# TRI-ML/sdflabel

Measured on AMD Instinct MI355X. Metric: rendered rays/sec (fwd+bwd), higher is better.
Workload: dtype f32; 1 GPU; BASELINE configs[1]: one 256x256 crop(s) per GPU, DeepSDF 8x512 on a 40^3 grid, fwd+bwd to yaw/trans/latent, decoder re-evaluated every step; crops_per_gpu=1, rays_per_crop=65536, grid_points=64000, surfels=2751, front_facing=763, parallelism=crop-parallel x1

## Files before the change

### include/sdfr.h

```cpp
#ifndef SDFR_H
#define SDFR_H

#include <stdint.h>

#ifdef __cplusplus
extern "C" {
#endif

#define SDFR_OK 0
#define SDFR_E_INVALID (-1)
#define SDFR_E_HIP (-2)
#define SDFR_E_UNSUPPORTED (-3)

#define SDFR_MAX_LAYERS 16
#define SDFR_TRACE_LEVELS 6
#define SDFR_TRACE_COUNTERS 32

#define SDFR_VERSION 415

int sdfr_version(void);
int sdfr_build_flags(void);
const char* sdfr_last_error(void);

typedef struct sdfr_decoder sdfr_decoder;

int sdfr_decoder_create(sdfr_decoder** out, int n_lin, const int* in_dim, const int* out_dim,
                        const int* inj_n, const int* inj_off, const float* const* h_W, const float* const* h_b,
                        const float* const* h_ln_w, const float* const* h_ln_b, int n_inputs, int use_tanh, int device);
int sdfr_decoder_destroy(sdfr_decoder* dec);
int64_t sdfr_decoder_macs(const sdfr_decoder* dec);

int sdfr_mlp_forward(const sdfr_decoder* dec, const float* inputs, int64_t n, float* sdf,
                     uint32_t* mask_ws ,
                     void* stream);
int sdfr_grid_tile_order(int D, int32_t* out);
int sdfr_mlp_forward_ordered(const sdfr_decoder* dec, const float* inputs, int64_t n, float* sdf, uint32_t* mask_ws, const int32_t* order,
                             int64_t order_rows, void* stream);
int sdfr_mlp_forward_f16(const sdfr_decoder* dec, const float* inputs, int64_t n, float* sdf, uint32_t* mask_ws, void* stream);

int sdfr_mlp_forward_f16_counted(const sdfr_decoder* dec, const float* inputs, int64_t n_max, const int32_t* n_dev, float* sdf, uint32_t* mask_ws,
                                 void* stream);

int sdfr_mlp_forward_split(const sdfr_decoder* dec, const float* inputs, int64_t n, float* sdf, uint32_t* mask_ws, void* stream);
int sdfr_mlp_forward_split_counted(const sdfr_decoder* dec, const float* inputs, int64_t n_max, const int32_t* n_dev, float* sdf, void* stream);
int64_t sdfr_decoder_mask_words(const sdfr_decoder* dec, int64_t n);

int sdfr_mlp_jacobian(const sdfr_decoder* dec, const float* inputs, int64_t rows_per_crop, int B,
                      const int32_t* idx, int cap, const int32_t* cnt, float* J, float* sdf_sel,
                      const float* sdf_full ,
                      const uint32_t* mask_ws ,
                      int mask_from_f16 ,
                      void* stream);
// ... 340 lines not shown
                     const int32_t* windows, const int64_t* poff, int64_t P, const int32_t* triangle, const int32_t* owner, const int32_t* scene,
                     const int32_t* boxes, const int64_t* qoff, int64_t Q, const double* paint, const double* light, int S, const int32_t* bg_index,
                     const uint8_t* bg, int NBG, const int32_t* ramp, int B, int W, int H, const double* K, float z_min, uint8_t* rgb, int32_t* flags,
                     void* stream);

int64_t sdfr_mesh_sdf_ws_bytes(int B, int64_t N, int64_t T);
int sdfr_mesh_sdf(const float* vertices, int64_t V, const int32_t* faces, int64_t T, const int64_t* voff, const int64_t* toff,
                  const float* points, int64_t N, const int64_t* qoff, int B, int want_sign, void* ws, int64_t ws_bytes, float* sdf, float* dist,
                  double* d2, int32_t* nearest, double* winding, int32_t* flags, void* stream);
int64_t sdfr_mesh_surface_ws_bytes(int B, int64_t T);
int sdfr_mesh_surface_points(const float* vertices, int64_t V, const int32_t* faces, int64_t T, const int64_t* voff, const int64_t* toff,
                             const float* uniforms, int64_t S, const int64_t* soff, int B, void* ws, int64_t ws_bytes, float* points,
                             int32_t* triangle, int32_t* flags, void* stream);

int sdfr_debug_set_trace(void* device_buffer);

#ifdef __cplusplus
}
#endif
#endif
```

### sdflabel_amd/_lib.py

```python
import ctypes
import os
from ctypes import POINTER, c_char_p, c_float, c_int, c_int32, c_int64, c_void_p

_HERE = os.path.dirname(os.path.abspath(__file__))
LIB_PATH = os.environ.get("SDFR_LIB") or os.path.join(_HERE, "lib", "libsdfr_hip.so")

ABI_VERSION = 415
_lib = None

_PROTOS = {
    "sdfr_version": (c_int, []),
    "sdfr_build_flags": (c_int, []),
    "sdfr_last_error": (c_char_p, []),
    "sdfr_debug_set_trace": (c_int, [c_void_p]),
    "sdfr_mlp_forward_counted": (c_int, [c_void_p, c_void_p, c_int64, c_void_p, c_void_p, c_int, c_void_p]),
    "sdfr_trace_setup": (c_int, [c_void_p, c_void_p, c_void_p, c_int, c_int, c_int, c_int, c_float, c_float, c_void_p, c_void_p, c_void_p,
                                 c_void_p, c_void_p, c_void_p, c_int, c_void_p]),
    "sdfr_trace_setup2": (c_int, [c_void_p, c_void_p, c_void_p, c_int, c_int, c_int, c_int, c_float, c_float, c_void_p, c_void_p, c_void_p,
                                  c_void_p, c_void_p, c_void_p, c_int, c_void_p, c_void_p, c_void_p]),
    "sdfr_trace_cone": (c_int, [c_void_p, c_void_p, c_void_p, c_void_p, c_int, c_int, c_int, c_int, c_float, c_float, c_float, c_int, c_int,
                                c_int, c_float, c_int, c_void_p, c_void_p, c_void_p, c_void_p, c_void_p, c_void_p, c_void_p, c_void_p, c_void_p,
                                c_void_p, c_void_p]),
    "sdfr_trace_step": (c_int, [c_void_p, c_void_p, c_void_p, c_int, c_int, c_int, c_float, c_void_p, c_void_p, c_int, c_int64, c_void_p,
                                c_void_p, c_void_p, c_void_p, c_void_p, c_void_p, c_void_p, c_void_p, c_void_p]),
    "sdfr_trace_march": (c_int, [c_void_p, c_void_p, c_void_p, c_void_p, c_int, c_int, c_int, c_int, c_float, c_int, c_int, c_int, c_void_p, c_int,
                                 c_float, c_float, c_int, c_void_p, c_void_p, c_void_p, c_void_p, c_void_p, c_void_p, c_void_p, c_void_p,
                                 c_void_p, c_void_p, c_void_p, c_void_p, c_void_p, c_void_p]),
    "sdfr_trace_pool": (c_int, []),
    "sdfr_trace_hits": (c_int, [c_void_p, c_void_p, c_void_p, c_int, c_int, c_int, c_int, c_void_p, c_void_p, c_void_p, c_void_p, c_void_p, c_void_p]),
# ... 29 lines not shown
                                      c_void_p, c_void_p, c_void_p, c_void_p, c_void_p, c_void_p, c_void_p, c_void_p, c_void_p, c_void_p, c_void_p,
                                      c_void_p, c_void_p]),
    "sdfr_loss_2d_r": (c_int, [c_void_p, c_void_p, c_int, c_void_p, c_int, c_int, c_float, c_float, c_float, c_void_p, c_void_p, c_void_p,
                               c_void_p, c_void_p]),
    "sdfr_prefilter_audit_select": (c_int, [c_void_p, c_void_p, c_int64, c_int, c_int, c_int, c_void_p, c_void_p, c_void_p, c_void_p, c_int, c_void_p]),
    "sdfr_prefilter_audit_check": (c_int, [c_void_p, c_void_p, c_void_p, c_void_p, c_int, c_int64, c_int, c_float, c_void_p, c_void_p, c_void_p,
                                           c_void_p, c_void_p]),
    "sdfr_scale_net": (c_int, [c_void_p, c_int, c_void_p, c_void_p, c_void_p, c_void_p, c_void_p, c_void_p, c_void_p, c_void_p]),
    "sdfr_decoder_create": (c_int, [POINTER(c_void_p), c_int, POINTER(c_int), POINTER(c_int), POINTER(c_int), POINTER(c_int),
                                    POINTER(c_void_p), POINTER(c_void_p), POINTER(c_void_p), POINTER(c_void_p), c_int, c_int, c_int]),
    "sdfr_decoder_destroy": (c_int, [c_void_p]),
    "sdfr_decoder_macs": (c_int64, [c_void_p]),
    "sdfr_mlp_forward": (c_int, [c_void_p, c_void_p, c_int64, c_void_p, c_void_p, c_void_p]),
    "sdfr_grid_tile_order": (c_int, [c_int, c_void_p]),
    "sdfr_mlp_forward_ordered": (c_int, [c_void_p, c_void_p, c_int64, c_void_p, c_void_p, c_void_p, c_int64, c_void_p]),
    "sdfr_mlp_forward_f16": (c_int, [c_void_p, c_void_p, c_int64, c_void_p, c_void_p, c_void_p]),
    "sdfr_mlp_forward_f16_counted": (c_int, [c_void_p, c_void_p, c_int64, c_void_p, c_void_p, c_void_p, c_void_p]),
    "sdfr_mlp_forward_split": (c_int, [c_void_p, c_void_p, c_int64, c_void_p, c_void_p, c_void_p]),
    "sdfr_mlp_forward_split_counted": (c_int, [c_void_p, c_void_p, c_int64, c_void_p, c_void_p, c_void_p]),
    "sdfr_decoder_mask_words": (c_int64, [c_void_p, c_int64]),
    "sdfr_mlp_jacobian": (c_int, [c_void_p, c_void_p, c_int64, c_int, c_void_p, c_int, c_void_p, c_void_p, c_void_p, c_void_p,
                                  c_void_p, c_int, c_void_p]),
    "sdfr_band_select": (c_int, [c_void_p, c_int64, c_int, c_float, c_void_p, c_int, c_void_p, c_void_p, c_void_p, c_void_p]),
    "sdfr_band_select_margin": (c_int, [c_void_p, c_int64, c_int, c_float, c_void_p, c_void_p, c_int, c_void_p, c_void_p, c_void_p, c_void_p]),
    "sdfr_prefilter_guard": (c_int, [c_void_p, c_void_p, c_void_p, c_int64, c_int, c_int, c_void_p, c_void_p, c_void_p, c_void_p, c_void_p]),
    "sdfr_prefilter_plan": (c_int, [c_void_p, c_int64, c_int, c_int, c_int, c_float, c_void_p, c_void_p, c_void_p, c_void_p, c_int, c_void_p, c_void_p,
                                    c_void_p]),
    "sdfr_mlp_forward_f16_skip": (c_int, [c_void_p, c_void_p, c_int64, c_void_p, c_void_p, c_int64, c_void_p]),
    "sdfr_band_select_skip": (c_int, [c_void_p, c_int64, c_int, c_float, c_void_p, c_void_p, c_void_p, c_int, c_void_p, c_void_p, c_void_p, c_void_p]),
    "sdfr_prefilter_guard2": (c_int, [c_void_p, c_void_p, c_void_p, c_int64, c_int, c_int, c_void_p, c_void_p, c_void_p, c_void_p, c_void_p, c_void_p]),
# ... 188 lines not shown
    return torch._C._cuda_getCurrentRawStream(torch._C._cuda_getDevice())


class _NoGuard:
    def __enter__(self):
        return None

    def __exit__(self, *exc):
        return False


_NO_GUARD = _NoGuard()


TRAFFIC_SOURCES = {
    "traffic_mlp_forward.json": ("mlp_kernel.h", "kc_slots.h", "mlp.hip", "mlp_fwd32.hip"),
    "traffic_splat.json": ("splat.hip", "splat_bbox.h"),
    "traffic_sphere_step.json": ("trace.hip",),
}


def source_sha16(names):
    import hashlib
    h = hashlib.sha256()
    for n in names:
        with open(os.path.join(os.path.dirname(os.path.abspath(__file__)), "csrc", n), "rb") as f:
            h.update(n.encode() + b"\0" + f.read())
    return h.hexdigest()[:16]


def stored_traffic(root, name):
# ... 49 lines not shown
```

### sdflabel_amd/batch.py

```python
import math
import os

import torch

from . import _lib
from .grid import Grid3D

_DIAM_DISC = 0.04
_DEPTH_CONSTANT = 150.0
P, ck = _lib.ptr, _lib.check


class BatchRenderer:
    def __init__(self, decoder, density, K, resolution_px, batch, cap=None, device="cuda", threshold=0.03, output_nocs=True,
                 max_pixels=None, max_side=None, candidate_reuse=None):
        dev = torch.device(device)
        if dev.type != "cuda":
            raise _lib.SdfrError("BatchRenderer runs on the GPU only")
        self.dev, self.B = dev, int(batch)
        self._f = lambda *shape: torch.zeros(shape, dtype=torch.float32, device=dev)
        self._i = lambda *shape: torch.zeros(shape, dtype=torch.int32, device=dev)
        self.W, self.H = int(resolution_px[0]), int(resolution_px[1])
        self.thr = float(threshold)
        self.nocs_mode = 1 if output_nocs else 0
# ... 1 lines not shown
            raise NotImplementedError("BatchRenderer composites NOCS colours (the optimizer's configuration)")
        self.decoder = decoder
        prec = getattr(decoder, "mlp_precision", torch.float32)
        self.f16, self.split, self.prefilter = prec == torch.float16, prec == "float32_split", prec == "float32_prefilter"
        self.margin = float(getattr(decoder, "prefilter_margin", 0.005))
        self.handle = decoder.handle(dev)
        self.fused = bool(getattr(decoder, "fused_launches", True))
        self.L, self.NI = decoder.latent_size, decoder.latent_size + 3
        self.grid = Grid3D(density, dev).points.detach().contiguous()
        self.G = self.grid.shape[0]
        self.fwd_order = None
        if prec == torch.float32 and self.handle.hp == 512 and not self.handle.has_ln and self.G == int(density) ** 3:
            order = torch.empty(self.G, dtype=torch.int32)
            ck(_lib.lib().sdfr_grid_tile_order(int(density), P(order)), "sdfr_grid_tile_order")
            self.fwd_order = order.to(dev)
        self.cap = int(cap) if cap is not None else max(256, self.G // 8)
        self._init_extents(K, max_pixels, max_side)
        self._alloc_common()
        want_reuse = bool(getattr(decoder, "candidate_reuse", False)) if candidate_reuse is None else bool(candidate_reuse)
        self.creuse = (self.f16 or prec == torch.float32) and want_reuse and self.handle.hp == 512 and not self.handle.has_ln
        self.reuse_off_reason = None
        if want_reuse and not self.creuse:
            self.reuse_off_reason = "candidate reuse needs a float16 / float32 decoder of padded width 512 without LayerNorm"
        if self.prefilter:
            self._setup_prefilter(decoder)
        elif self.creuse:
            self._setup_candidate_reuse(decoder)
        self.mode = "prefilter" if self.prefilter else ("creuse" if self.creuse else "plain")
        self.guarded = self.prefilter or self.creuse
        self.n_full = self._i(self.B) if self.guarded else None
# ... 236 lines not shown
        return {"color": self.color, "mask": self.mask, "depth": self.depth, "normals": self.nimg, "xyzf": self.xyzf, "nf": self.fcnt, "n": self.cnt}

    def _params_stage(self, L, st, frozen):
        B, G = self.B, self.G
        if self.creuse and self.fused and not frozen:
            ck(L.sdfr_params_plan(P(self.yaw), P(self.trans), P(self.latent), self.L, P(self.grid), G, B, P(self.inputs), P(self.pose), P(self.latnorm),
                                  self.lipschitz_plan, P(self.margin_dev), P(self.max_dev), P(self.lat_ref), P(self.age), self.max_reuse, P(self.reuse_flag),
                                  P(self.n_full), st), "sdfr_params_plan")
        else:
            ck(L.sdfr_params_forward(P(self.yaw), P(self.trans), P(self.latent), self.L, P(self.grid), G, B, None if frozen else P(self.inputs),
                                     P(self.pose), P(self.latnorm), st), "sdfr_params_forward")

    def _decoder_plain(self, L, st, mlp_events, events):
        B, G, cap = self.B, self.G, self.cap
        fwd = L.sdfr_mlp_forward_f16 if self.f16 else (L.sdfr_mlp_forward_split if self.split else L.sdfr_mlp_forward)
        if self.fwd_order is not None and os.environ.get("SDFR_FWD_ORDER", "1") != "0":
            ck(L.sdfr_mlp_forward_ordered(self.handle.h, P(self.inputs), B * G, P(self.sdf), P(self.mask_ws), P(self.fwd_order), G, st),
               "sdfr_mlp_forward_ordered")
        else:
            ck(fwd(self.handle.h, P(self.inputs), B * G, P(self.sdf), P(self.mask_ws), st), fwd.__name__)
        if mlp_events is not None:
            mlp_events[1].record()
        ck(L.sdfr_band_select_ex(P(self.sdf), G, B, self.thr, None, None, P(self.idx), cap, P(self.cnt), None, P(self.scratch), P(self.over), 1, st),
           "sdfr_band_select_ex")
        if "jacobian" in events:
            events["jacobian"][0].record()
        ck(L.sdfr_mlp_jacobian(self.handle.h, P(self.inputs), G, B, P(self.idx), cap, P(self.cnt), P(self.J), P(self.sdf_band), P(self.sdf),
                               P(self.mask_ws), 2 if self.f16 else 0, st), "sdfr_mlp_jacobian")
        if "jacobian" in events:
            events["jacobian"][1].record()

# ... 241 lines not shown
```

### sdflabel_amd/csrc/mlp.hip

```cpp
#include "mlp_kernel.h"
#include <algorithm>
#include <cmath>
#include <stdlib.h>
#include <string.h>
#include <vector>


#define SDFR_DEVICE_CHECK(d, what)                                                                                                          \
    do {                                                                                                                                    \
        int cur_ = -1;                                                                                                                      \
        SDFR_HIP_CHECK(hipGetDevice(&cur_));                                                                                                \
        SDFR_REQUIRE(cur_ == (d)->device, "%s: the decoder's weights live on device %d but the current device (the launch stream's) is %d: " \
                     "create one decoder handle per device", what, (d)->device, cur_);                                                      \
    } while (0)

extern "C" int sdfr_decoder_create(sdfr_decoder** out, int n_lin, const int* in_dim, const int* out_dim,
                                   const int* inj_n, const int* inj_off, const float* const* h_W,
                                   const float* const* h_b, const float* const* h_ln_w, const float* const* h_ln_b, int n_inputs,
                                   int use_tanh, int device) {
    SDFR_REQUIRE(out && in_dim && out_dim && inj_n && inj_off && h_W && h_b, "sdfr_decoder_create: NULL argument");
    SDFR_REQUIRE(n_lin >= 2 && n_lin <= SDFR_MAX_LAYERS, "sdfr_decoder_create: n_lin=%d outside [2,%d]", n_lin, SDFR_MAX_LAYERS);
    SDFR_REQUIRE(out_dim[n_lin - 1] == 1, "sdfr_decoder_create: last layer must have out_dim 1 (got %d)", out_dim[n_lin - 1]);
    SDFR_REQUIRE(in_dim[0] == n_inputs && inj_n[0] == 0, "sdfr_decoder_create: layer 0 must consume exactly the input row");
    int width = 0;
// ... 115 lines not shown
        P.kcompact = finite ? 1 : 0;
    }
    if (!Wkj.empty()) {
        SDFR_HIP_CHECK(hipMalloc(&d->d_Wkj, Wkj.size() * sizeof(float)));
        SDFR_HIP_CHECK(hipMemcpy(d->d_Wkj, Wkj.data(), Wkj.size() * sizeof(float), hipMemcpyHostToDevice));
        P.Wkj = d->d_Wkj;
        P.jcompact = finite ? 1 : 0;
    }
    P.Wf = d->d_Wf; P.Wb = d->d_Wb; P.Wh = d->d_Wh; P.Ws = d->d_Ws; P.Wbh = d->d_Wbh; P.bias = d->d_bias; P.w_last = d->d_wlast; P.fwd_np = 2;
    *out = d;
    return SDFR_OK;
}

static unsigned long long* g_trace = nullptr;
extern "C" int sdfr_debug_set_trace(void* device_buffer) { g_trace = (unsigned long long*)device_buffer; return SDFR_OK; }

extern "C" int sdfr_decoder_destroy(sdfr_decoder* d) {
    if (!d) return SDFR_OK;
    void* bufs[] = {d->d_Wf, d->d_Wb, d->d_Wk, d->d_Wkj, d->d_Wh, d->d_Ws, d->d_Wbh, d->d_bias, d->d_wlast, d->d_lng, d->d_lnb, d->ln_ws};
    for (void* b : bufs) (void)hipFree(b);
    delete d;
    return SDFR_OK;
}

extern "C" int64_t sdfr_decoder_macs(const sdfr_decoder* d) { return d ? d->macs : 0; }

static void mask_geometry(int HP, int* ft, int* nt) {
    if (HP == 128) { *ft = 1; *nt = 256; }
    else if (HP == 256) { *ft = 2; *nt = 256; }
    else { *ft = 2; *nt = 512; }
// ... 1 lines not shown

extern "C" int64_t sdfr_decoder_mask_words(const sdfr_decoder* d, int64_t n) {
    if (!d || n <= 0) return 0;
    int ft, nt;
    mask_geometry(d->HP, &ft, &nt);
    return ((n + 127) / 128) * 2 * (int64_t)(d->n_lin - 1) * ft * nt;
}

extern "C" int sdfr_mlp_forward(const sdfr_decoder* d, const float* inputs, int64_t n, float* sdf, uint32_t* mask_ws, void* stream) {
    SDFR_REQUIRE(d && inputs && sdf, "sdfr_mlp_forward: NULL argument");
    SDFR_DEVICE_CHECK(d, "sdfr_mlp_forward");
    SDFR_REQUIRE(n >= 0 && n < (int64_t)1 << 31, "sdfr_mlp_forward: n=%lld out of range", (long long)n);
    if (n == 0) return SDFR_OK;
    MlpParams P = d->proto;
    P.inputs = inputs; P.n = n; P.sdf = sdf; P.maskbuf = mask_ws; P.trace = g_trace;
    const int grid = sdfr_cdiv(n, 64);
    if (d->has_ln) sdfr_launch_ln(P, d->HP, false, grid, 1, (hipStream_t)stream);
    else if (d->HP == 512) sdfr_launch_fwd_f32_512(P, n, mask_ws != nullptr, (hipStream_t)stream);
    else sdfr_launch_small(P, d->HP, mask_ws ? 1 : 0, grid, 1, (hipStream_t)stream);
    SDFR_LAUNCH_CHECK();
    return SDFR_OK;
}

extern "C" int sdfr_grid_tile_order(int D, int32_t* out) {
    SDFR_REQUIRE(out, "sdfr_grid_tile_order: NULL argument");
    SDFR_REQUIRE(D >= 1 && D <= 1024, "sdfr_grid_tile_order: D=%d outside [1,1024]", D);
    int64_t j = 0;
    for (int bx = 0; bx < D; bx += 4)
        for (int by = 0; by < D; by += 4)
            for (int bz = 0; bz < D; bz += 4)
// ... 5 lines not shown

extern "C" int sdfr_mlp_forward_ordered(const sdfr_decoder* d, const float* inputs, int64_t n, float* sdf, uint32_t* mask_ws, const int32_t* order,
                                        int64_t order_rows, void* stream) {
    SDFR_REQUIRE(d && inputs && sdf && order, "sdfr_mlp_forward_ordered: NULL argument");
    SDFR_REQUIRE(n >= 0 && n < (int64_t)1 << 31, "sdfr_mlp_forward_ordered: n=%lld out of range", (long long)n);
    SDFR_REQUIRE(order_rows > 0, "sdfr_mlp_forward_ordered: order_rows=%lld must be positive", (long long)order_rows);
    SDFR_REQUIRE(n % order_rows == 0, "sdfr_mlp_forward_ordered: n=%lld is not a multiple of order_rows=%lld", (long long)n, (long long)order_rows);
    SDFR_REQUIRE(d->HP == 512 && !d->has_ln, "sdfr_mlp_forward_ordered: needs a float32 decoder of padded width 512 without LayerNorm (this one: %d%s)",
                 d->HP, d->has_ln ? ", LayerNorm" : "");
    SDFR_REQUIRE(!mask_ws || ((n + 127) / 128) * 128 * (int64_t)(d->n_lin - 1) < (int64_t)1 << 31,
                 "sdfr_mlp_forward_ordered: n=%lld rows with masks of %d layers exceed the kernel's line index", (long long)n, d->n_lin - 1);
    SDFR_DEVICE_CHECK(d, "sdfr_mlp_forward_ordered");
    if (n == 0) return SDFR_OK;
    MlpParams P = d->proto;
    P.inputs = inputs; P.n = n; P.sdf = sdf; P.maskbuf = mask_ws; P.trace = g_trace;
    sdfr_launch_fwd_f32_512_ordered(P, n, order, order_rows, (hipStream_t)stream);
    SDFR_LAUNCH_CHECK();
    return SDFR_OK;
}

#ifndef SDFR_COUNTED_TILE16_ROWS
#define SDFR_COUNTED_TILE16_ROWS 4096
#endif
extern "C" int sdfr_mlp_forward_counted(const sdfr_decoder* d, const float* inputs, int64_t n_max, const int32_t* n_dev, float* sdf, int half,
                                        void* stream) {
    SDFR_REQUIRE(d && inputs && sdf && n_dev, "sdfr_mlp_forward_counted: NULL argument");
    SDFR_DEVICE_CHECK(d, "sdfr_mlp_forward_counted");
    SDFR_REQUIRE(n_max >= 0 && n_max < (int64_t)1 << 31, "sdfr_mlp_forward_counted: n_max=%lld out of range", (long long)n_max);
    SDFR_REQUIRE(!half || (d->HP == 512 && !d->has_ln), "sdfr_mlp_forward_counted: half operands need a 512-wide decoder without LayerNorm");
    if (n_max == 0) return SDFR_OK;
    MlpParams P = d->proto;
    P.inputs = inputs; P.n = n_max; P.sdf = sdf; P.maskbuf = nullptr; P.n_dev = n_dev; P.trace = g_trace;
// ... 211 lines not shown
```

### sdflabel_amd/csrc/mlp_kernel.h

```cpp
#pragma once
#include "sdfr_common.h"
#include "kc_slots.h"
#include "kcj_slots.h"
#include <math.h>
#include <type_traits>

typedef float f32x16 __attribute__((ext_vector_type(16)));
typedef float f32x4 __attribute__((ext_vector_type(4)));
typedef _Float16 h16;
typedef h16 h16x8 __attribute__((ext_vector_type(8)));
typedef h16 h16x4 __attribute__((ext_vector_type(4)));

struct MlpLayer {
    int in_dim, out_dim;
    int inj_n, inj_off;
    int kp_f, kp_b, kp_h;
    int off_f, off_b, off_h;
    int kp_bh, off_bh;
    int kp_s, off_s;
    int ln;
};

struct MlpParams {
    const float4* Wf;
// ... 50 lines not shown
    int32_t* t_next_cnt;
    int32_t* t_next_pix;
    float4* t_next_lam;
    const float* t_far;
    const float* t_pose;
    const float* t_Kinv;
    float* t_hit_lam;
    float* t_hit_sdf;
    int t_W, t_H, t_steps;
    const int32_t* t_wh; int t_PS;
    float t_eps, t_sigma;
    unsigned long long* t_evals;
    int32_t* t_unresolved;
    const float* Wkj;
    int jcompact;
};

struct sdfr_decoder {
    int device;
    int n_lin, n_inputs, use_tanh, HP;
    float4* d_Wf;
    float4* d_Wb;
    float* d_Wk;
    float* d_Wkj;
    void* d_Wh;
    void* d_Ws;
    void* d_Wbh;
    float* d_lng;
    float* d_lnb;
    int has_ln;
    mutable float4* ln_ws;
// ... 136 lines not shown
    const int lane = tid & 63;
    const int lp = lane % MS;
    const int lg = lane / MS;
    const int NI = P.n_inputs;

#ifdef SDFR_MLP_TRACE
#define SDFR_STAMP(l, i)                                                                                                   \
    do {                                                                                                                   \
        if (P.trace && blockIdx.x == 0 && blockIdx.y == 0 && lane == 0 && wave < 8)                                        \
            P.trace[(wave * SDFR_MAX_LAYERS + (l)) * 5 + (i)] = __builtin_amdgcn_s_memtime();                              \
    } while (0)
#else
#define SDFR_STAMP(l, i) do { } while (0)
#endif
    SDFR_STAMP(8, 0);
    int* tile_slot = reinterpret_cast<int*>(gy) + 1;
    int p_iter = 0, p_live = 0;
    bool p_compact = false;
    if constexpr (PERSIST) {
        if (P.crop_cnt && P.n_crops <= PT) {
            if (tid == 0) {
                int acc_ = 0;
                for (int c = 0; c < P.n_crops; ++c) {
                    const int64_t cc = min((int64_t)P.crop_cnt[c], P.crop_rows);
                    acc_ += (int)((cc + PT - 1) / PT);
                    slots[c] = acc_;
                }
                tile_slot[1] = acc_;
            }
            __syncthreads();
// ... 87 lines not shown
                const int64_t c = r0 / P.crop_rows, sc = r0 - c * P.crop_rows + tid;
                const bool live = sc < (int64_t)P.crop_cnt[c];
                rows[tid] = (int)(c * P.gather_rows + (live ? P.gather_idx[c * P.crop_rows + sc] : 0));
            }
        } else
        if constexpr (ORDER) {
            if (tid < PT) {
                const int64_t G = P.gather_rows, j = r0 + tid, c = j / G;
                const int o = tid < n_valid ? P.gather_idx[j - c * G] : -1;
                const bool ok = o >= 0 && (int64_t)o < G;
                const int64_t row = ok ? c * G + o : (r0 / G) * G;
                rows[tid] = (int)row;
                slots[tid] = ok ? (int)row : -1;
                reinterpret_cast<int*>(gy)[tid] = ok ? (int)((row >> 7) * P.n_mfma * 128 + (row & 127)) : -1;
            }
        } else
        if (tid < PT) rows[tid] = TAIL ? (int)((int64_t)blockIdx.x * PT + tid) : (int)(r0 + (tid < n_valid ? tid : 0));
    }
    const int RT = TAIL ? P.t_rt : 1;
    const int KMAX = TAIL ? PT / RT : 1;
    auto pass_k = [&](int s) {
        int k = 1;
        for (int i = 0; i < P.t_nlv; ++i) k = (s >= P.t_lv_from[i]) ? P.t_lv_k[i] : k;
        return min(KMAX, k);
    };
    int t_gp = 0, t_left = 0, t_pass = 0;
    bool t_act = false;
    float4 t_st = make_float4(0.f, 0.f, 1.f, 0.f);
    float t_farl = 0.f, t_idn = 1.f, t_ox = 0.f, t_oy = 0.f, t_oz = 0.f, t_dx = 0.f, t_dy = 0.f, t_dz = 0.f;
    unsigned long long t_ev = 0ull;
// ... 623 lines not shown
                        *reinterpret_cast<float2*>(act_e + dl + sdfr_kcm_lane_dword(sdfr_kcd_row_reg(f * RG * 4 + r), 0)) =
                            make_float2(acc[f][0][r], acc[f][NP - 1][r]);
            }
            {
                const int q = lp;
                if ((kc_w[lg] >> q) & 1u) {
                    const int j = fbase + sdfr_kcd_feature(0, q, lg);
                    reinterpret_cast<int*>(kc_list4)[sdfr_kc_slot(off + sdfr_kc_rank(kc_w[0], kc_w[1], q, lg))] = sdfr_kcd_entry(j);
                }
            }
            const int padded = sdfr_kc_padded(tot);
            if (sdfr_kcm_pads(wave)) {
                if (lane < padded - tot) reinterpret_cast<int*>(kc_list4)[sdfr_kc_slot(tot + lane)] = sdfr_kcd_pad_entry();
            }
            kc_n = padded;
        };
        auto epilogue = [&](auto inj_tag) {
            constexpr bool INJ = decltype(inj_tag)::value;
            int elane = ((fbase / KV + lg) * PT + lp) * KV;
            if constexpr (KC) asm volatile("" : "+v"(elane));
#pragma unroll
            for (int f = 0; f < FT; ++f)
#pragma unroll
                for (int rg = 0; rg < RG; ++rg) {
                    const int j0 = feat0(f, rg);
                    const float4 b4 = lnl ? make_float4(0.f, 0.f, 0.f, 0.f) : b4s[f][rg];
#pragma unroll
                    for (int p = 0; p < NP; ++p) {
                        const int pt = p * MS + lp;
                        float v[4];
// ... 180 lines not shown
                        P.t_hit_lam[t_gp] = pj;
                        P.t_hit_sdf[t_gp] = vj;
                        t_act = false;
                    } else {
                        const float qn = (prev > 0.f) ? fminf(fmaxf(rj / prev, 0.5f), P.t_qmax) : 1.f;
                        const float l2 = pj + vj / t_idn;
                        t_st.y = rj; t_st.z = qn;
                        if ((l2 < t_farl) && (vj == vj)) t_st.x = l2;
                        else t_act = false;
                    }
                  }
                }
            } else if constexpr (ORDER) {
                const int row = slots[tid];
                if (row >= 0 && (!P.skip || !P.skip[row / P.skip_rows])) P.sdf[row] = o;
            } else {
                if (tid < n_valid) {
                    const int64_t row = (int64_t)tile * PT + tid;
                    if (!P.skip || !P.skip[row / P.skip_rows]) P.sdf[row] = o;
                }
            }
        }
    }
    if constexpr (TAIL) {
        --t_left;
        if (tid == 0) *t_more = 0;
        __syncthreads();
        if (t_act && t_left > 0) *t_more = 1;
        __syncthreads();
        if (*t_more == 0) break;
        ++t_pass;
        tail_rows(pass_k(P.t_step0 + t_pass), false);
        __syncthreads();
        build_operand();
        __syncthreads();
    }
    } while (TAIL);
    if constexpr (TAIL) {
// ... 425 lines not shown
                        if (slots[pt] < 0) continue;
#pragma unroll
                        for (int i = 0; i < 4; ++i)
                            if (j0 + i < NI) atomicAdd(P.J + (int64_t)slots[pt] * NI + j0 + i, acc[f][p][rg * 4 + i]);
                    }
                }
        }
    }
    }
    } while (TAIL || PERSIST);
}


void sdfr_launch_fwd_f32_512(const MlpParams& P, int64_t n, bool save_masks, hipStream_t s);
void sdfr_launch_fwd_f32_512_ordered(const MlpParams& P, int64_t n, const int32_t* order, int64_t order_rows, hipStream_t s);
int sdfr_fwd_f32_512_np();
void sdfr_launch_fwd_f16_512(const MlpParams& P, int64_t n, bool save_masks, hipStream_t s);
void sdfr_launch_fwd_f16_512_half_tiles(const MlpParams& P, int64_t n, hipStream_t s);
int sdfr_fwd_f16_512_np();
void sdfr_launch_fwd_split_512(const MlpParams& P, int64_t n, bool save_masks, hipStream_t s);
void sdfr_launch_jac_f32_512(const MlpParams& P, int cap, int B, bool from_masks, hipStream_t s);
void sdfr_launch_jac_f32_512_recompute32(const MlpParams& P, int cap, int B, hipStream_t s);
void sdfr_launch_fwd_f32_512_tile16(const MlpParams& P, int64_t n, hipStream_t s);
void sdfr_launch_jac_f16_512(const MlpParams& P, int cap, int B, hipStream_t s);
void sdfr_launch_fwd_f16_512_tile16(const MlpParams& P, int64_t n, hipStream_t s);
void sdfr_launch_fwd_f16_512_tile64(const MlpParams& P, int64_t n, hipStream_t s);
void sdfr_launch_tail_f32_512(const MlpParams& P, int64_t n_rays, int spec_k, hipStream_t s);
void sdfr_launch_jac_f16_512_many(const MlpParams& P, int cap, int B, hipStream_t s);
void sdfr_launch_tail_f16_512(const MlpParams& P, int64_t n_rays, int spec_k, hipStream_t s);
void sdfr_launch_pool_f16_skip(const MlpParams& P, int64_t n, hipStream_t s);
// ... 9 lines not shown
```

Measured before the change: 54.46 million rays/s.

## Reorder grid tiles by measured per-tile cost for longest-first scheduling

```diff
diff --git a/include/sdfr.h b/include/sdfr.h
--- a/include/sdfr.h
+++ b/include/sdfr.h
@@ -16,7 +16,7 @@
 #define SDFR_TRACE_LEVELS 6
 #define SDFR_TRACE_COUNTERS 32
 
-#define SDFR_VERSION 415
+#define SDFR_VERSION 416
 
 int sdfr_version(void);
 int sdfr_build_flags(void);
@@ -36,6 +36,10 @@
 int sdfr_grid_tile_order(int D, int32_t* out);
 int sdfr_mlp_forward_ordered(const sdfr_decoder* dec, const float* inputs, int64_t n, float* sdf, uint32_t* mask_ws, const int32_t* order,
                              int64_t order_rows, void* stream);
+int64_t sdfr_mlp_balance_bytes(int64_t order_rows);
+int sdfr_mlp_balance_init(void* state, const int32_t* order, int64_t order_rows, void* stream);
+int sdfr_mlp_forward_balanced(const sdfr_decoder* dec, const float* inputs, int64_t n, float* sdf, uint32_t* mask_ws, void* state,
+                              int64_t order_rows, void* stream);
 int sdfr_mlp_forward_f16(const sdfr_decoder* dec, const float* inputs, int64_t n, float* sdf, uint32_t* mask_ws, void* stream);
 
 int sdfr_mlp_forward_f16_counted(const sdfr_decoder* dec, const float* inputs, int64_t n_max, const int32_t* n_dev, float* sdf, uint32_t* mask_ws,
@@ -406,6 +410,7 @@
                              int32_t* triangle, int32_t* flags, void* stream);
 
 int sdfr_debug_set_trace(void* device_buffer);
+int sdfr_debug_set_tile_trace(void* device_buffer, int64_t tiles);
 
 #ifdef __cplusplus
 }
diff --git a/sdflabel_amd/_lib.py b/sdflabel_amd/_lib.py
--- a/sdflabel_amd/_lib.py
+++ b/sdflabel_amd/_lib.py
@@ -5,7 +5,7 @@
 _HERE = os.path.dirname(os.path.abspath(__file__))
 LIB_PATH = os.environ.get("SDFR_LIB") or os.path.join(_HERE, "lib", "libsdfr_hip.so")
 
-ABI_VERSION = 415
+ABI_VERSION = 416
 _lib = None
 
 _PROTOS = {
@@ -13,6 +13,7 @@
     "sdfr_build_flags": (c_int, []),
     "sdfr_last_error": (c_char_p, []),
     "sdfr_debug_set_trace": (c_int, [c_void_p]),
+    "sdfr_debug_set_tile_trace": (c_int, [c_void_p, c_int64]),
     "sdfr_mlp_forward_counted": (c_int, [c_void_p, c_void_p, c_int64, c_void_p, c_void_p, c_int, c_void_p]),
     "sdfr_trace_setup": (c_int, [c_void_p, c_void_p, c_void_p, c_int, c_int, c_int, c_int, c_float, c_float, c_void_p, c_void_p, c_void_p,
                                  c_void_p, c_void_p, c_void_p, c_int, c_void_p]),
@@ -72,6 +73,9 @@
     "sdfr_mlp_forward": (c_int, [c_void_p, c_void_p, c_int64, c_void_p, c_void_p, c_void_p]),
     "sdfr_grid_tile_order": (c_int, [c_int, c_void_p]),
     "sdfr_mlp_forward_ordered": (c_int, [c_void_p, c_void_p, c_int64, c_void_p, c_void_p, c_void_p, c_int64, c_void_p]),
+    "sdfr_mlp_balance_bytes": (c_int64, [c_int64]),
+    "sdfr_mlp_balance_init": (c_int, [c_void_p, c_void_p, c_int64, c_void_p]),
+    "sdfr_mlp_forward_balanced": (c_int, [c_void_p, c_void_p, c_int64, c_void_p, c_void_p, c_void_p, c_int64, c_void_p]),
     "sdfr_mlp_forward_f16": (c_int, [c_void_p, c_void_p, c_int64, c_void_p, c_void_p, c_void_p]),
     "sdfr_mlp_forward_f16_counted": (c_int, [c_void_p, c_void_p, c_int64, c_void_p, c_void_p, c_void_p, c_void_p]),
     "sdfr_mlp_forward_split": (c_int, [c_void_p, c_void_p, c_int64, c_void_p, c_void_p, c_void_p]),
@@ -290,7 +294,7 @@
 
 
 TRAFFIC_SOURCES = {
-    "traffic_mlp_forward.json": ("mlp_kernel.h", "kc_slots.h", "mlp.hip", "mlp_fwd32.hip"),
+    "traffic_mlp_forward.json": ("mlp_kernel.h", "kc_slots.h", "tile_balance.h", "mlp.hip", "mlp_fwd32.hip", "mlp_balance.hip"),
     "traffic_splat.json": ("splat.hip", "splat_bbox.h"),
     "traffic_sphere_step.json": ("trace.hip",),
 }
diff --git a/sdflabel_amd/batch.py b/sdflabel_amd/batch.py
--- a/sdflabel_amd/batch.py
+++ b/sdflabel_amd/batch.py
@@ -39,6 +39,10 @@
             order = torch.empty(self.G, dtype=torch.int32)
             ck(_lib.lib().sdfr_grid_tile_order(int(density), P(order)), "sdfr_grid_tile_order")
             self.fwd_order = order.to(dev)
+            lib = _lib.lib()
+            self.fwd_balance = torch.empty(int(lib.sdfr_mlp_balance_bytes(self.G)) // 4, dtype=torch.int32, device=dev)
+            with _lib.guard(dev):
+                ck(lib.sdfr_mlp_balance_init(P(self.fwd_balance), P(self.fwd_order), self.G, _lib.stream_ptr()), "sdfr_mlp_balance_init")
         self.cap = int(cap) if cap is not None else max(256, self.G // 8)
         self._init_extents(K, max_pixels, max_side)
         self._alloc_common()
@@ -305,7 +309,10 @@
     def _decoder_plain(self, L, st, mlp_events, events):
         B, G, cap = self.B, self.G, self.cap
         fwd = L.sdfr_mlp_forward_f16 if self.f16 else (L.sdfr_mlp_forward_split if self.split else L.sdfr_mlp_forward)
-        if self.fwd_order is not None and os.environ.get("SDFR_FWD_ORDER", "1") != "0":
+        if self.fwd_order is not None and os.environ.get("SDFR_FWD_ORDER", "1") != "0" and os.environ.get("SDFR_FWD_BALANCE", "1") != "0":
+            ck(L.sdfr_mlp_forward_balanced(self.handle.h, P(self.inputs), B * G, P(self.sdf), P(self.mask_ws), P(self.fwd_balance), G, st),
+               "sdfr_mlp_forward_balanced")
+        elif self.fwd_order is not None and os.environ.get("SDFR_FWD_ORDER", "1") != "0":
             ck(L.sdfr_mlp_forward_ordered(self.handle.h, P(self.inputs), B * G, P(self.sdf), P(self.mask_ws), P(self.fwd_order), G, st),
                "sdfr_mlp_forward_ordered")
         else:
diff --git a/sdflabel_amd/csrc/mlp.hip b/sdflabel_amd/csrc/mlp.hip
--- a/sdflabel_amd/csrc/mlp.hip
+++ b/sdflabel_amd/csrc/mlp.hip
@@ -153,6 +153,13 @@
 
 static unsigned long long* g_trace = nullptr;
 extern "C" int sdfr_debug_set_trace(void* device_buffer) { g_trace = (unsigned long long*)device_buffer; return SDFR_OK; }
+static unsigned long long* g_tile_trace = nullptr;
+static int64_t g_tile_trace_cap = 0;
+extern "C" int sdfr_debug_set_tile_trace(void* device_buffer, int64_t tiles) {
+    g_tile_trace = tiles > 0 ? (unsigned long long*)device_buffer : nullptr;
+    g_tile_trace_cap = g_tile_trace ? tiles : 0;
+    return SDFR_OK;
+}
 
 extern "C" int sdfr_decoder_destroy(sdfr_decoder* d) {
     if (!d) return SDFR_OK;
@@ -184,6 +191,7 @@
     if (n == 0) return SDFR_OK;
     MlpParams P = d->proto;
     P.inputs = inputs; P.n = n; P.sdf = sdf; P.maskbuf = mask_ws; P.trace = g_trace;
+    P.tile_trace = g_tile_trace; P.tile_trace_cap = g_tile_trace_cap;
     const int grid = sdfr_cdiv(n, 64);
     if (d->has_ln) sdfr_launch_ln(P, d->HP, false, grid, 1, (hipStream_t)stream);
     else if (d->HP == 512) sdfr_launch_fwd_f32_512(P, n, mask_ws != nullptr, (hipStream_t)stream);
@@ -219,8 +227,56 @@
     if (n == 0) return SDFR_OK;
     MlpParams P = d->proto;
     P.inputs = inputs; P.n = n; P.sdf = sdf; P.maskbuf = mask_ws; P.trace = g_trace;
+    P.tile_trace = g_tile_trace; P.tile_trace_cap = g_tile_trace_cap;
     sdfr_launch_fwd_f32_512_ordered(P, n, order, order_rows, (hipStream_t)stream);
     SDFR_LAUNCH_CHECK();
+    return SDFR_OK;
+}
+
+extern "C" int64_t sdfr_mlp_balance_bytes(int64_t order_rows) {
+    return order_rows > 0 && order_rows < (int64_t)1 << 31 ? sdfr_tb_state_words(order_rows) * 4 : 0;
+}
+
+extern "C" int sdfr_mlp_balance_init(void* state, const int32_t* order, int64_t order_rows, void* stream) {
+    SDFR_REQUIRE(state && order, "sdfr_mlp_balance_init: NULL argument");
+    SDFR_REQUIRE(order_rows > 0 && order_rows < (int64_t)1 << 31, "sdfr_mlp_balance_init: order_rows=%lld out of range", (long long)order_rows);
+    int cur = -1;
+    hipPointerAttribute_t attr;
+    SDFR_HIP_CHECK(hipGetDevice(&cur));
+    SDFR_HIP_CHECK(hipPointerGetAttributes(&attr, state));
+    SDFR_REQUIRE(attr.type == hipMemoryTypeDevice && attr.device == cur,
+                 "sdfr_mlp_balance_init: the state must be device memory of the current device %d (the launch stream's); it is %s of device %d", cur,
+                 attr.type == hipMemoryTypeDevice ? "memory" : "not device memory", attr.device);
+    sdfr_launch_tile_balance_init((int32_t*)state, order, order_rows, (hipStream_t)stream);
+    SDFR_LAUNCH_CHECK();
+    return SDFR_OK;
+}
+
+extern "C" int sdfr_mlp_forward_balanced(const sdfr_decoder* d, const float* inputs, int64_t n, float* sdf, uint32_t* mask_ws, void* state,
+                                         int64_t order_rows, void* stream) {
+    SDFR_REQUIRE(d && inputs && sdf && state, "sdfr_mlp_forward_balanced: NULL argument");
+    SDFR_REQUIRE(n >= 0 && n < (int64_t)1 << 31, "sdfr_mlp_forward_balanced: n=%lld out of range", (long long)n);
+    SDFR_REQUIRE(order_rows > 0, "sdfr_mlp_forward_balanced: order_rows=%lld must be positive", (long long)order_rows);
+    SDFR_REQUIRE(n % order_rows == 0, "sdfr_mlp_forward_balanced: n=%lld is not a multiple of order_rows=%lld", (long long)n, (long long)order_rows);
+    SDFR_REQUIRE(d->HP == 512 && !d->has_ln, "sdfr_mlp_forward_balanced: needs a float32 decoder of padded width 512 without LayerNorm (this one: %d%s)",
+                 d->HP, d->has_ln ? ", LayerNorm" : "");
+    SDFR_REQUIRE(!mask_ws || ((n + 127) / 128) * 128 * (int64_t)(d->n_lin - 1) < (int64_t)1 << 31,
+                 "sdfr_mlp_forward_balanced: n=%lld rows with masks of %d layers exceed the kernel's line index", (long long)n, d->n_lin - 1);
+    SDFR_DEVICE_CHECK(d, "sdfr_mlp_forward_balanced");
+    if (n == 0) return SDFR_OK;
+    int32_t* st = (int32_t*)state;
+    const bool ranked = sdfr_tb_ranked(order_rows);
+    MlpParams P = d->proto;
+    P.inputs = inputs; P.n = n; P.sdf = sdf; P.maskbuf = mask_ws; P.trace = g_trace;
+    P.tile_trace = g_tile_trace; P.tile_trace_cap = g_tile_trace_cap;
+    P.tile_cost = ranked ? st + sdfr_tb_cost_word(order_rows) : nullptr;
+    P.tile_at = st + sdfr_tb_at_word(order_rows);
+    sdfr_launch_fwd_f32_512_ordered(P, n, st + sdfr_tb_order_word(order_rows), order_rows, (hipStream_t)stream);
+    SDFR_LAUNCH_CHECK();
+    if (ranked) {
+        sdfr_launch_tile_balance(st, order_rows, (hipStream_t)stream);
+        SDFR_LAUNCH_CHECK();
+    }
     return SDFR_OK;
 }
 
diff --git a/sdflabel_amd/csrc/mlp_balance.hip b/sdflabel_amd/csrc/mlp_balance.hip
--- /dev/null
+++ b/sdflabel_amd/csrc/mlp_balance.hip
@@ -0,0 +1,63 @@
+#include <hip/hip_runtime.h>
+#include "sdfr_common.h"
+#include "tile_balance.h"
+
+constexpr int TB_NT = 256, TB_WAVES = TB_NT / 64;
+
+__global__ __launch_bounds__(256) void sdfr_tile_balance_init_kernel(int32_t* __restrict__ state, const int32_t* __restrict__ order, int64_t order_rows) {
+    const int64_t i = (int64_t)blockIdx.x * blockDim.x + threadIdx.x;
+    const int64_t T = sdfr_tb_chunks(order_rows);
+    if (i < 3 * T + SDFR_TB_CTL) state[i] = (i < 2 * T || i >= 3 * T) ? 0 : (int32_t)(i - 2 * T);
+    if (i < order_rows) {
+        const int32_t o = order[i];
+        state[sdfr_tb_order_word(order_rows) + i] = o;
+        state[sdfr_tb_fixed_word(order_rows) + i] = o;
+    }
+}
+
+__global__ __launch_bounds__(TB_NT) void sdfr_tile_balance_kernel(int32_t* __restrict__ state, int64_t order_rows) {
+    __shared__ int32_t cost[SDFR_TB_MAX_CHUNKS];
+    __shared__ int last_reader;
+    const int T = (int)sdfr_tb_chunks(order_rows), full = (int)sdfr_tb_full_chunks(order_rows);
+    int32_t* g_cost = state + sdfr_tb_cost_word(order_rows);
+    int32_t* g_last = state + sdfr_tb_last_word(order_rows);
+    int32_t* g_at = state + sdfr_tb_at_word(order_rows);
+    int32_t* ctl = state + sdfr_tb_ctl_word(order_rows);
+    int32_t* order = state + sdfr_tb_order_word(order_rows);
+    const int32_t* fixed = state + sdfr_tb_fixed_word(order_rows);
+    const int tid = threadIdx.x, lane = tid & 63, wave = tid >> 6;
+    const int c = (int)blockIdx.x * TB_WAVES + wave;
+    const int64_t i = (int64_t)c * SDFR_TB_CHUNK + lane;
+    const bool moves = c < T && i < order_rows;
+    const int32_t entry = moves ? fixed[i] : 0;
+    for (int k = tid; k < T; k += TB_NT) cost[k] = g_cost[k];
+    __syncthreads();
+    if (c < T) {
+        int r = c;
+        if (c < full) {
+            r = sdfr_tb_rank_part(cost, full, c, lane, 64);
+#pragma unroll
+            for (int d = 32; d >= 1; d >>= 1) r += __shfl_xor(r, d, 64);
+        }
+        if (lane == 0) {
+            g_last[c] = cost[c];
+            g_at[r] = c;
+        }
+        if (moves) order[sdfr_tb_dest(c, r, lane, full)] = entry;
+    }
+    if (tid == 0) last_reader = atomicAdd(ctl, 1) == (int)gridDim.x - 1 ? 1 : 0;
+    __syncthreads();
+    if (last_reader) {
+        for (int k = tid; k < T; k += TB_NT) g_cost[k] = 0;
+        if (tid == 0) ctl[0] = 0;
+    }
+}
+
+void sdfr_launch_tile_balance_init(int32_t* state, const int32_t* order, int64_t order_rows, hipStream_t s) {
+    const int64_t head = 3 * sdfr_tb_chunks(order_rows) + SDFR_TB_CTL, n = order_rows > head ? order_rows : head;
+    hipLaunchKernelGGL(sdfr_tile_balance_init_kernel, dim3(sdfr_cdiv(n, 256)), dim3(256), 0, s, state, order, order_rows);
+}
+
+void sdfr_launch_tile_balance(int32_t* state, int64_t order_rows, hipStream_t s) {
+    hipLaunchKernelGGL(sdfr_tile_balance_kernel, dim3(sdfr_cdiv(sdfr_tb_chunks(order_rows), TB_WAVES)), dim3(TB_NT), 0, s, state, order_rows);
+}
diff --git a/sdflabel_amd/csrc/mlp_kernel.h b/sdflabel_amd/csrc/mlp_kernel.h
--- a/sdflabel_amd/csrc/mlp_kernel.h
+++ b/sdflabel_amd/csrc/mlp_kernel.h
@@ -2,6 +2,7 @@
 #include "sdfr_common.h"
 #include "kc_slots.h"
 #include "kcj_slots.h"
+#include "tile_balance.h"
 #include <math.h>
 #include <type_traits>
 
@@ -88,7 +89,12 @@
     int32_t* t_unresolved;
     const float* Wkj;
     int jcompact;
+    int32_t* tile_cost;
+    const int32_t* tile_at;
+    unsigned long long* tile_trace;
+    int64_t tile_trace_cap;
 };
+#define SDFR_TILE_TRACE_WORDS 6
 
 struct sdfr_decoder {
     int device;
@@ -255,6 +261,16 @@
 #define SDFR_STAMP(l, i) do { } while (0)
 #endif
     SDFR_STAMP(8, 0);
+#ifdef SDFR_MLP_TRACE
+    const bool tt_on = !JAC && !TAIL && P.tile_trace && tid == 0 && blockIdx.y == 0 && (int64_t)blockIdx.x < P.tile_trace_cap;
+    if (tt_on) {
+        unsigned long long* tt = P.tile_trace + (int64_t)blockIdx.x * SDFR_TILE_TRACE_WORDS;
+        tt[0] = __builtin_amdgcn_s_memtime();
+        tt[1] = __builtin_amdgcn_s_memrealtime();
+        tt[4] = ((unsigned long long)__builtin_amdgcn_s_getreg(20 | (31 << 11)) << 32) | (unsigned long long)__builtin_amdgcn_s_getreg(4 | (31 << 11));
+        tt[5] = blockIdx.x;
+    }
+#endif
     int* tile_slot = reinterpret_cast<int*>(gy) + 1;
     int p_iter = 0, p_live = 0;
     bool p_compact = false;
@@ -372,6 +388,8 @@
                 slots[tid] = ok ? (int)row : -1;
                 reinterpret_cast<int*>(gy)[tid] = ok ? (int)((row >> 7) * P.n_mfma * 128 + (row & 127)) : -1;
             }
+            static_assert(!ORDER || PT <= 64, "ORDER: rows[127] is the tile's cost");
+            if (tid == 0) rows[127] = 0;
         } else
         if (tid < PT) rows[tid] = TAIL ? (int)((int64_t)blockIdx.x * PT + tid) : (int)(r0 + (tid < n_valid ? tid : 0));
     }
@@ -1025,6 +1043,9 @@
                 if (lane < padded - tot) reinterpret_cast<int*>(kc_list4)[sdfr_kc_slot(tot + lane)] = sdfr_kcd_pad_entry();
             }
             kc_n = padded;
+            if constexpr (ORDER) {
+                if (tid == 0) __hip_atomic_fetch_add(rows + 127, sdfr_tb_layer_cost(tot), __ATOMIC_RELAXED, __HIP_MEMORY_SCOPE_WORKGROUP);
+            }
         };
         auto epilogue = [&](auto inj_tag) {
             constexpr bool INJ = decltype(inj_tag)::value;
@@ -1235,6 +1256,10 @@
             } else if constexpr (ORDER) {
                 const int row = slots[tid];
                 if (row >= 0 && (!P.skip || !P.skip[row / P.skip_rows])) P.sdf[row] = o;
+                if (P.tile_cost && tid == 0) {
+                    const int place = sdfr_tb_place_of_tile(tile, P.gather_rows);
+                    atomicAdd(P.tile_cost + sdfr_tb_cost_index(P.tile_at[place], place, P.gather_rows), rows[127]);
+                }
             } else {
                 if (tid < n_valid) {
                     const int64_t row = (int64_t)tile * PT + tid;
@@ -1243,6 +1268,13 @@
             }
         }
     }
+#ifdef SDFR_MLP_TRACE
+    if (tt_on) {
+        unsigned long long* tt = P.tile_trace + (int64_t)blockIdx.x * SDFR_TILE_TRACE_WORDS;
+        tt[2] = __builtin_amdgcn_s_memtime();
+        tt[3] = __builtin_amdgcn_s_memrealtime();
+    }
+#endif
     if constexpr (TAIL) {
         --t_left;
         if (tid == 0) *t_more = 0;
@@ -1698,6 +1730,8 @@
 
 void sdfr_launch_fwd_f32_512(const MlpParams& P, int64_t n, bool save_masks, hipStream_t s);
 void sdfr_launch_fwd_f32_512_ordered(const MlpParams& P, int64_t n, const int32_t* order, int64_t order_rows, hipStream_t s);
+void sdfr_launch_tile_balance_init(int32_t* state, const int32_t* order, int64_t order_rows, hipStream_t s);
+void sdfr_launch_tile_balance(int32_t* state, int64_t order_rows, hipStream_t s);
 int sdfr_fwd_f32_512_np();
 void sdfr_launch_fwd_f16_512(const MlpParams& P, int64_t n, bool save_masks, hipStream_t s);
 void sdfr_launch_fwd_f16_512_half_tiles(const MlpParams& P, int64_t n, hipStream_t s);
diff --git a/sdflabel_amd/csrc/tile_balance.h b/sdflabel_amd/csrc/tile_balance.h
--- /dev/null
+++ b/sdflabel_amd/csrc/tile_balance.h
@@ -0,0 +1,55 @@
+#pragma once
+#include <stdint.h>
+#include "kc_slots.h"
+#if defined(__HIPCC__) || defined(__CUDACC__)
+#define SDFR_TB_HD __host__ __device__ __forceinline__
+#else
+#define SDFR_TB_HD inline
+#endif
+
+constexpr int SDFR_TB_CHUNK = 64;
+constexpr int SDFR_TB_MAX_CHUNKS = 4096;
+constexpr int SDFR_TB_CTL = 4;
+
+SDFR_TB_HD int64_t sdfr_tb_chunks(int64_t order_rows) { return (order_rows + SDFR_TB_CHUNK - 1) / SDFR_TB_CHUNK; }
+SDFR_TB_HD int64_t sdfr_tb_full_chunks(int64_t order_rows) { return order_rows / SDFR_TB_CHUNK; }
+SDFR_TB_HD bool sdfr_tb_ranked(int64_t order_rows) { return sdfr_tb_chunks(order_rows) <= SDFR_TB_MAX_CHUNKS; }
+SDFR_TB_HD int sdfr_tb_place_of_tile(int64_t tile, int64_t order_rows) {
+    return (int)((uint32_t)tile * (uint32_t)SDFR_TB_CHUNK % (uint32_t)order_rows / (uint32_t)SDFR_TB_CHUNK);
+}
+SDFR_TB_HD int sdfr_tb_layer_cost(int survivors) { return sdfr_kc_padded(survivors); }
+
+SDFR_TB_HD int64_t sdfr_tb_cost_word(int64_t order_rows) { (void)order_rows; return 0; }
+SDFR_TB_HD int64_t sdfr_tb_last_word(int64_t order_rows) { return sdfr_tb_chunks(order_rows); }
+SDFR_TB_HD int64_t sdfr_tb_at_word(int64_t order_rows) { return 2 * sdfr_tb_chunks(order_rows); }
+SDFR_TB_HD int64_t sdfr_tb_ctl_word(int64_t order_rows) { return 3 * sdfr_tb_chunks(order_rows); }
+SDFR_TB_HD int64_t sdfr_tb_order_word(int64_t order_rows) { return 3 * sdfr_tb_chunks(order_rows) + SDFR_TB_CTL; }
+SDFR_TB_HD int64_t sdfr_tb_fixed_word(int64_t order_rows) { return sdfr_tb_order_word(order_rows) + order_rows; }
+SDFR_TB_HD int64_t sdfr_tb_state_words(int64_t order_rows) { return sdfr_tb_order_word(order_rows) + 2 * order_rows; }
+SDFR_TB_HD int sdfr_tb_cost_index(int at_place, int place, int64_t order_rows) {
+    return (uint32_t)at_place < (uint32_t)sdfr_tb_chunks(order_rows) ? at_place : place;
+}
+
+SDFR_TB_HD int sdfr_tb_rank_part(const int32_t* cost, int full, int i, int first, int step) {
+    const int32_t ci = cost[i];
+    int r = 0;
+    for (int j = first; j < full; j += step) {
+        const int32_t cj = cost[j];
+        r += (cj > ci || (cj == ci && j < i)) ? 1 : 0;
+    }
+    return r;
+}
+SDFR_TB_HD int sdfr_tb_rank(const int32_t* cost, int full, int i) { return sdfr_tb_rank_part(cost, full, i, 0, 1); }
+SDFR_TB_HD int64_t sdfr_tb_dest(int64_t chunk, int rank, int e, int64_t full) {
+    return (chunk < full ? (int64_t)rank : chunk) * SDFR_TB_CHUNK + e;
+}
+
+inline void sdfr_tb_next_order_host(const int32_t* cost, const int32_t* fixed, int32_t* next, int32_t* at, int64_t order_rows) {
+    const int64_t T = sdfr_tb_chunks(order_rows), full = sdfr_tb_full_chunks(order_rows);
+    for (int64_t c = 0; c < T; ++c) {
+        const int rank = (c < full && sdfr_tb_ranked(order_rows)) ? sdfr_tb_rank(cost, (int)full, (int)c) : (int)c;
+        const int64_t n = c < full ? SDFR_TB_CHUNK : order_rows - full * SDFR_TB_CHUNK;
+        at[rank] = (int32_t)c;
+        for (int e = 0; e < n; ++e) next[sdfr_tb_dest(c, rank, e, full)] = fixed[c * SDFR_TB_CHUNK + e];
+    }
+}
```

Result: faster. 56.08 million rays/s, median of 6 (+3.0%).
